# Healthcare-Robotics/mr-gan

Measured on AMD Instinct MI355X. Metric: GAN train steps/sec (labeled+unlabeled+G) at batch 4096, higher is better.
Workload: dtype bf16; 1 GPU; BASELINE configs[1]: synthetic N=65536 x D=512, K=6, batch 4096 per GPU, labeled 100/class; one step = D sub-step (3B rows) + G sub-step (2B rows) + both Adam updates; global_batch=4096, rows_per_gpu=4096, parallelism=single, batch_statistics=n/a, launch=hipGraph replay

## Files before the change

### include/mrgan_abi.h

```cpp
#ifndef MRGAN_ABI_H
#define MRGAN_ABI_H

#include <stddef.h>
#include <stdint.h>

#ifdef __cplusplus
extern "C" {
#endif

typedef struct mrgan_handle mrgan_handle;
typedef void* mrgan_stream;

enum { MRGAN_F32 = 0, MRGAN_BF16 = 1, MRGAN_FP8 = 2 };
enum { MRGAN_NET_G = 0, MRGAN_NET_D = 1 };
enum {
    MRGAN_FLAG_SYNC_STATS = 1,
    MRGAN_FLAG_FLAT_GRADS = 2,
    MRGAN_FLAG_GRAPH      = 4,
    MRGAN_FLAG_GRAD_BF16  = 8,
    MRGAN_FLAG_GAUSS_NOISE = 16
};

#define MRGAN_MAX_CLASSES 32
#define MRGAN_MAX_MODELS 16
// ... 85 lines not shown
    const float* x_unl_dev; const int32_t* idx_unl_dev;
    const float* z_dev;
    int64_t ld_x_lab, ld_x_unl;
    int64_t x_lab_model_stride, idx_lab_model_stride, labels_model_stride;
    int64_t x_unl_model_stride, idx_unl_model_stride, z_model_stride;
    int32_t stream_mode, reserved;
} mrgan_disc_group_args;
typedef struct mrgan_gen_group_args {
    const float* x_unl_dev; const int32_t* idx_unl_dev;
    const float* z_dev;
    int64_t ld_x_unl;
    int64_t x_unl_model_stride, idx_unl_model_stride, z_model_stride;
    int32_t stream_mode, reserved;
} mrgan_gen_group_args;
int mrgan_disc_step_group(mrgan_handle* h, const mrgan_disc_group_args* a, float* out3_host, mrgan_stream stream);
int mrgan_gen_step_group(mrgan_handle* h, const mrgan_gen_group_args* a, float* out1_host, mrgan_stream stream);
int mrgan_train_pair_group(mrgan_handle* h, const mrgan_disc_group_args* d, const mrgan_gen_group_args* g, mrgan_stream stream);

enum {
    MRGAN_TUNE_CHAIN = 0,
    MRGAN_TUNE_KC_CFG = 1,
    MRGAN_TUNE_KS_GROUP = 4,
    MRGAN_TUNE_PAIR_GEN = 5,
    MRGAN_TUNE_HEAD_MFMA = 6
};
int mrgan_set_tuning(mrgan_handle* h, int knob, int value);

enum {
    MRGAN_REGION_BN_STATS = 0,
    MRGAN_REGION_FM_MOMENTS = 1,
    MRGAN_REGION_BN_BWD = 2,
    MRGAN_REGION_GRAD_D = 3,
    MRGAN_REGION_GRAD_G = 4,
    MRGAN_REGION_WORKSPACE = 5,
    MRGAN_REGION_GRAD_D_BF16 = 6,
    MRGAN_REGION_GRAD_G_BF16 = 7,
    MRGAN_REGION_TAIL_D = 8,
    MRGAN_REGION_TAIL_G = 9
};
int mrgan_region(mrgan_handle* h, int region, void** ptr_dev, size_t* bytes);

int mrgan_eval_error(mrgan_handle* h, const float* x_dev, const int32_t* idx_dev, int64_t ld_x,
                     const int32_t* labels_dev, int64_t n, float* err_host, mrgan_stream stream);
int mrgan_predict_logits(mrgan_handle* h, const float* x_dev, const int32_t* idx_dev, int64_t ld_x, int64_t n,
                         float* logits_dev, mrgan_stream stream);

int mrgan_read_metrics(mrgan_handle* h, float* out8_host, int reset, mrgan_stream stream);
// ... 11 lines not shown
```

### include/mrgan_debug.h

```cpp
#ifndef MRGAN_DEBUG_H
#define MRGAN_DEBUG_H

#include "mrgan_abi.h"

#ifdef __cplusplus
extern "C" {
#endif

int mrgan_debug_noise(mrgan_handle* h, uint32_t site, uint32_t seg, uint32_t step, uint32_t row0, int rows, int cols,
                      float* out_dev, mrgan_stream stream);
int mrgan_debug_tr_probe(uint16_t* out1024_dev, mrgan_stream stream);
int mrgan_debug_ablate(mrgan_handle* h, int bits);
int mrgan_debug_buffer(mrgan_handle* h, int kind, int l, void** ptr_dev, int* rows_per_seg, int* ld, int* elem_size);
int mrgan_debug_gemm_time(int op, int m, int n, int k, int nbatch, int splits, int reps, int ablate, int kc_cfg, float* avg_us);

typedef struct mrgan_debug_gemm_desc {
    int32_t dtype, op, m, n, k, nbatch, splits;
    int32_t kchunk;
    int32_t kc_cfg;
    int32_t tune_bits;
    int32_t seg_stride, seg_rows;
    const void* a; int64_t a_bs, a_si, a_sk;
    const void* b; int64_t b_bs, b_sk, b_sj;
    int32_t act, n_valid;
    const float* bias;
    void* out; int64_t out_bs; int32_t ldo;
    float sigma; uint32_t site, seg0; int32_t seg_step; uint32_t iter_step, row0;
    uint32_t iter;
    uint64_t seed;
    uint16_t* mask; int64_t mask_bs; int32_t ldm;
    const void* h; int64_t h_bs; int32_t ldh;
    int32_t cs_mode; float* cs1; float* cs2; int32_t ldcs;
    const float* bn_mu; const float* bn_rstd;
    float* slab; int64_t slab_stride;
    void* q8; int64_t q8_bs; int32_t ldq8;
    void* q8t; int64_t q8t_bs; int32_t ldq8t;
    const void* slot_a; const void* slot_b; void* slot_o;
    int32_t gauss;
} mrgan_debug_gemm_desc;
typedef struct mrgan_debug_fold { const float* src; float* dst; int64_t stride; int32_t nsrc, n, ngroups; } mrgan_debug_fold;
int mrgan_debug_gemm_launch(const mrgan_debug_gemm_desc* d, int count, int grouped, const mrgan_debug_fold* fold,
                            char* kname, int kname_len, mrgan_stream stream);

int mrgan_debug_gemm_fp8(int m, int n, int k, const float* a_dev, const float* b_dev, const float* bias_dev, int act, float scale_a,
                         float scale_b, float* out_dev, int reps, float* avg_us, int kc_cfg, mrgan_stream stream);

int mrgan_debug_quant8(const void* src, int64_t src_bs, int ld, int rows, int cols, int nb, int prow, void* dst, int64_t dst_bs, int ldd,
                       void* dstt, int64_t dstt_bs, int lddt, void* slot_dev, int fmt, mrgan_stream stream);
int mrgan_debug_fp8_update_scales(void* slots_dev, int n, mrgan_stream stream);


typedef struct mrgan_debug_stage_seg {
    const float* src; const int32_t* idx; int64_t ld;
    int32_t rows, cols, cols_pad;
    void* out; int32_t ldo;
    float sigma; uint32_t site, seg;
    int32_t gen, stream; uint32_t iter_off;
    int32_t models; int64_t src_ms, idx_ms, out_ms;
} mrgan_debug_stage_seg;
typedef struct mrgan_debug_stage_desc {
    int32_t dtype;
    mrgan_debug_stage_seg s[5]; int32_t nseg;
    uint64_t seed; uint32_t row0;
// ... 95 lines not shown
```

### mr_gan_amd/csrc/engine_debug.hip

```cpp
#include "engine_internal.h"

namespace mrgan {
int launch_tr_probe(unsigned short* out, hipStream_t s);
}

namespace {

template <typename T>
__global__ void to_f32_kernel(const T* src, long lds, float* dst, long ldd, int rows, int cols) {
    const int c = blockIdx.x * 64 + (threadIdx.x & 63), r = blockIdx.y * 4 + (threadIdx.x >> 6);
    if (r >= rows || c >= cols) return;
    dst[(long)r * ldd + c] = Elem<T>::to_f32(src[(long)r * lds + c]);
}

}

extern "C" {

int mrgan_debug_noise(mrgan_handle* h, uint32_t site, uint32_t seg, uint32_t step, uint32_t row0, int rows, int cols, float* out,
                      mrgan_stream stream) {
    if (!h || !out) return fail(-1, "null argument");
    if (h->gauss && (row0 & 1u)) return fail(-1, "debug_noise: a true-Gaussian handle draws row pairs, row0 must be even");
    CHK(launch_noise_debug(h->gauss, h->cfg.seed, site, seg, step, row0, rows, cols, out, (hipStream_t)stream));
    return 0;
// ... 211 lines not shown
        if (d.h && (d.ldh < d.n || (bf && (d.ldh % 8)))) return fail(-1, "debug_gemm_launch: ldh");
        if (d.mask && d.ldm < d.n) return fail(-1, "debug_gemm_launch: ldm >= n");
    }
    return 0;
}

int mrgan_debug_gemm_launch(const mrgan_debug_gemm_desc* d, int count, int grouped, const mrgan_debug_fold* fold,
                            char* kname, int kname_len, mrgan_stream stream) {
    if (!d || count < 1) return fail(-1, "null argument");
    if (kname && kname_len > 0) kname[0] = 0;
    hipStream_t s = (hipStream_t)stream;
    DevState* st = nullptr;
    DevState hst[2];
    memset(hst, 0, sizeof hst);
    hst[0].iter = hst[1].iter = d[0].iter;
    HIPCHK(hipMalloc((void**)&st, sizeof hst));
    hipError_t he = hipMemcpy(st, hst, sizeof hst, hipMemcpyHostToDevice);
    const char* name = "";
    int r = he == hipSuccess ? 0 : fail(-10, "hipMemcpy failed: %s", hipGetErrorString(he));
    if (!r && !grouped) {
        GemmArgs g;
        int epi = 0;
        if (count != 1) r = fail(-1, "debug_gemm_launch: one product per plain launch");
        if (!r) r = debug_gemm_args(d[0], st, g, epi);
        if (!r) {
            r = d[0].dtype == MRGAN_FP8    ? launch_gemm_fp8(epi, g, s, &name)
                : d[0].dtype == MRGAN_BF16 ? launch_gemm_bf16(epi, g, s, &name)
                                           : launch_gemm_f32(epi, g, s, &name);
            if (r) fail(r, "debug_gemm_launch: launch refused (%d)", r);
        }
    } else if (!r) {
        GemmArgs gs[KS_GROUP_MAX];
        for (int i = 0; i < count && i < KS_GROUP_MAX && !r; ++i) {
            int epi = 0;
            r = debug_gemm_args(d[i], st, gs[i], epi);
            if (!r && (epi != EPI_SLAB || d[i].dtype != MRGAN_BF16)) r = fail(-1, "debug_gemm_launch: grouped launches are bf16 weight gradients");
        }
        FoldJob fj;
        memset(&fj, 0, sizeof fj);
        if (!r && fold) {
            if (!fold->src || !fold->dst || fold->nsrc < 1 || fold->n < 1 || fold->ngroups < 1 || fold->stride < fold->n)
                r = fail(-1, "debug_gemm_launch: fold");
            fj.src = fold->src; fj.dst = fold->dst; fj.stride = fold->stride; fj.nsrc = fold->nsrc; fj.n = fold->n; fj.ngroups = fold->ngroups;
        }
        if (!r) {
            r = launch_gemm_bf16_dw_group(gs, count, s, &name, fold ? &fj : nullptr);
            if (r < 0) fail(r, "debug_gemm_launch: grouped launch failed (%d)", r);
        }
    }
    he = hipStreamSynchronize(s);
    hipFree(st);
    if (!r && he != hipSuccess) return fail(-10, "debug_gemm_launch: %s", hipGetErrorString(he));
    if (!r && kname && kname_len > 0) snprintf(kname, (size_t)kname_len, "%s", name);
    return r;
}

int mrgan_debug_quant8(const void* src, int64_t src_bs, int ld, int rows, int cols, int nb, int prow, void* dst, int64_t dst_bs, int ldd,
                       void* dstt, int64_t dstt_bs, int lddt, void* slot, int fmt, mrgan_stream stream) {
    if (!src || rows < 0 || rows > prow || cols < 1 || cols > ld || (fmt != FP8_E4M3 && fmt != FP8_E5M2)) return fail(-1, "debug_quant8: bad argument");
    if ((dst && ldd < cols) || (dstt && (dstt_bs < 0 || lddt < (int64_t)(nb - 1) * dstt_bs + prow))) return fail(-1, "debug_quant8: ldd >= cols, lddt >= nb batches of prow bytes");
    Quant8Args a;
    memset(&a, 0, sizeof a);
    a.src = (const __bf16*)src; a.src_bs = src_bs; a.ld = ld; a.rows = rows; a.cols = cols; a.nb = nb; a.prow = prow;
    a.dst = (unsigned char*)dst; a.dst_bs = dst_bs; a.ldd = ldd;
    a.dstt = (unsigned char*)dstt; a.dstt_bs = dstt_bs; a.lddt = lddt;
    a.slot = (Fp8Slot*)slot; a.fmt = fmt;
// ... 287 lines not shown
```

### mr_gan_amd/csrc/engine_state.hip

```cpp
#include <stdarg.h>

#include "engine_internal.h"

namespace mrgan {

thread_local std::string g_err;
int fail(int code, const char* fmt, ...) {
    char buf[512];
    va_list ap;
    va_start(ap, fmt);
    vsnprintf(buf, sizeof buf, fmt, ap);
    va_end(ap);
    g_err = buf;
    return code;
}

void set_gen_view(mrgan_handle* h, int seg) {
    h->g[1].q.xseg = seg;
    const int N1p = h->g[0].Np;
    h->zbuf = rowptr(h, h->zbuf_all, (long)seg * h->S, h->nzp);
    h->h1 = rowptr(h, h->h1_all, (long)seg * h->S, N1p);
    h->hbn = rowptr(h, h->hbn_all, (long)seg * h->S, N1p);
    h->h2 = rowptr(h, h->h2_all, (long)seg * h->S, h->g[1].Np);
    h->bn_mu = h->bn_mu_all + (size_t)seg * N1p;
// ... 449 lines not shown
    HIPCHK(hipStreamSynchronize((hipStream_t)stream));
    *it = st.iter;
    return 0;
}

int mrgan_set_iterations(mrgan_handle* h, uint32_t iterations, uint32_t batch_counter, mrgan_stream stream) {
    if (!h) return fail(-1, "null handle");
    hipLaunchKernelGGL(init_state_kernel, dim3(1), dim3(1), 0, (hipStream_t)stream, h->state, iterations, batch_counter,
                       h->cfg.lr, h->cfg.beta1, h->cfg.beta2);
    return 0;
}

int mrgan_set_tuning(mrgan_handle* h, int knob, int value) {
    if (!h) return fail(-1, "null handle");
    if (h->graph_exec) { hipGraphExecDestroy(h->graph_exec); h->graph_exec = nullptr; h->graph_ready = false; }
    switch (knob) {
        case MRGAN_TUNE_CHAIN: h->use_chain = value != 0 && h->chain_ok; break;
        case MRGAN_TUNE_KC_CFG:
            if (!kc_cfg_supported(value)) return fail(-1, "unsupported forward / dX tile config %d", value);
            h->tune_kc_cfg = value; break;
        case MRGAN_TUNE_KS_GROUP: h->tune_bits = (h->tune_bits & ~TUNE_BIT_NO_KS_GROUP) | (value ? 0 : TUNE_BIT_NO_KS_GROUP); break;
        case MRGAN_TUNE_PAIR_GEN: h->tune_pair_gen = value ? 1 : 0; break;
        case MRGAN_TUNE_HEAD_MFMA: h->head_wide = value != 0 && h->head_wide_ok; break;
        default: return fail(-1, "unknown tuning knob %d", knob);
    }
    return 0;
}

int mrgan_pair_hint(mrgan_handle* h, int on) {
    if (!h) return fail(-1, "null handle");
    h->pair_gen = on ? 1 : 0;
    return 0;
}

int mrgan_region(mrgan_handle* h, int region, void** ptr, size_t* bytes) {
    if (!h || !ptr || !bytes) return fail(-1, "null argument");
    const size_t n1 = (size_t)h->g[0].Np;
    switch (region) {
        case MRGAN_REGION_BN_STATS: *ptr = h->r_bn_stats; *bytes = 4 * n1 * 4; break;
        case MRGAN_REGION_FM_MOMENTS: *ptr = h->r_fm; *bytes = 2 * (size_t)h->Fp * 4; break;
        case MRGAN_REGION_BN_BWD: *ptr = h->r_bn_bwd; *bytes = 2 * n1 * 4; break;
        case MRGAN_REGION_GRAD_D: case MRGAN_REGION_GRAD_G: {
            if (h->flat16_d) return fail(-3, "region %d: the gradients of this handle travel as bfloat16 (MRGAN_FLAG_GRAD_BF16): "
                                             "all-reduce MRGAN_REGION_GRAD_*_BF16 and MRGAN_REGION_TAIL_*", region);
            const bool d = region == MRGAN_REGION_GRAD_D;
            *ptr = d ? h->flat_d : h->flat_g; *bytes = ((d ? h->flat_d_n : h->flat_g_n) + 4) * 4;
// ... 28 lines not shown
```

### mr_gan_amd/csrc/gemm.h

```cpp
#pragma once
#include <string.h>

#include <algorithm>

#include "common.h"

namespace mrgan {

enum { EPI_FWD = 0, EPI_DX = 1, EPI_SLAB = 2 };
enum { VAR_ACT_MASK = 3, VAR_NOISE = 4, VAR_MASK = 8, VAR_GAUSS = 16, VAR_DYN = 64 };


struct Epi {
    int act;
    int n_valid;
    const float* bias;
    void* out; long out_bs; int ldo;
    float sigma; uint32_t site; uint32_t seg0;
    int seg_step; uint32_t iter_step;
    uint32_t row0;
    uint64_t seed;
    int gauss;
    uint16_t* mask; long mask_bs; int ldm;
    const void* h; long h_bs; int ldh;
    int cs_mode; float* cs1; float* cs2; int ldcs;
    const float* bn_mu; const float* bn_rstd;
    float* slab; long slab_stride;
    const DevState* st;
// ... 344 lines not shown
                        const int c = wn * wcols + ni * 32 + lc;
                        lds[(wm * 2 + 0) * bn + c] = cs1[0][ni];
                        lds[(wm * 2 + 1) * bn + c] = cs2[0][ni];
                    }
                }
                __syncthreads();
                const int t = threadIdx.x;
                if (t < bn) {
                    float s1 = 0.f, s2 = 0.f;
#pragma unroll
                    for (int w = 0; w < WM; ++w) { s1 += lds[(w * 2 + 0) * bn + t]; s2 += lds[(w * 2 + 1) * bn + t]; }
                    if (col_blk + t < g.N && col_blk + t < e.ldcs) {
                        cs1p[prow0 * e.ldcs + col_blk + t] = s1;
                        if (e.cs_mode != CS_SUM) cs2p[prow0 * e.ldcs + col_blk + t] = s2;
                    }
                }
            }
        }
        EPI_STAMP(3);
    }
#undef EPI_STAMP
}

enum { TUNE_BIT_NO_KS_GROUP = 4 };
inline bool kc_cfg_supported(int cfg) {
    return cfg == -1 || cfg == 0 || cfg == 1 || cfg == 3 || cfg == 5 || cfg == 7 || cfg == 9;
}
constexpr int KS_GROUP_MAX = 6;
struct FoldJob { const float* src; float* dst; long stride; int nsrc, n, ngroups, blocks_x; long model_stride; };
struct KsGroup {
    int n;
    int blk_end[KS_GROUP_MAX];
    FoldJob fold;
    GemmArgs g[KS_GROUP_MAX];
};

int launch_gemm_f32(int epi, const GemmArgs& g, hipStream_t s, const char** kname = nullptr);
int launch_gemm_bf16(int epi, const GemmArgs& g, hipStream_t s, const char** kname = nullptr);
int launch_gemm_fp8(int epi, const GemmArgs& g, hipStream_t s, const char** kname = nullptr);
int launch_to_fp8(const float* src, long ld_src, unsigned char* dst, long ld_dst, int rows, int cols, int prow, int pcol, float scale,
                  int transpose, hipStream_t s);
struct Quant8Args {
    const __bf16* src; long src_bs; int ld; int rows, cols, nb;
    int prow;
    unsigned char* dst; long dst_bs; int ldd;
    unsigned char* dstt; long dstt_bs; int lddt;
    Fp8Slot* slot; int fmt;
};
int launch_quant8(const Quant8Args& a, hipStream_t s);
int launch_fp8_update_scales(Fp8Slot* slots, int n, hipStream_t s);
int launch_fp8_init_slots(Fp8Slot* slots, int n, const float* targets_dev, hipStream_t s);
int launch_gemm_bf16_dw_group(const GemmArgs* gs, int n, hipStream_t s, const char** kname = nullptr,
                              const FoldJob* fold = nullptr);

constexpr int GEMM_NO_HOLES = 1 << 30;
inline GemmArgs gemm_args(int M, int N, int K, int nbatch, int tile_rows) {
    GemmArgs g;
    memset(&g, 0, sizeof g);
// ... 64 lines not shown
```

### mr_gan_amd/csrc/gemm_bf16.hip

```cpp
#include <algorithm>
#include <cstring>
#include <string>

#include "gemm.h"
#include "lds_ring.h"

namespace mrgan {

namespace {
constexpr int BN = 128, BK = RING_BK;
constexpr int KS_PITCH = 320;
constexpr int KS_TILE_BYTES = 64 * KS_PITCH;

#ifdef MRGAN_STAMPS
struct KcStamps { unsigned long long acc[6], prev, epi[5]; };
#define KC_STAMPS_PARAM , KcStamps& stamps_
#define KC_STAMPS_ARG , stamps_
#else
#define KC_STAMPS_PARAM
#define KC_STAMPS_ARG
#endif
template <int EPI, int BM, int BNT, int WM, int WN, int NS, int VAR>
__device__ __forceinline__ void kc_tile(const GemmArgs& g, const int batch , const int model, const int tile_m, const int tile_n, char* lds KC_STAMPS_PARAM) {
    constexpr int NW = WM * WN;
// ... 131 lines not shown
    static const std::string name = "gemm_bf16_kc_kernel<" + std::to_string(EPI) + ", " + std::to_string(BM) + ", " +
                                    std::to_string(BNT) + ", " + std::to_string(WM) + ", " + std::to_string(WN) + ", " +
                                    std::to_string(NS) + ", " + std::to_string(VAR) + ">";
    g_last_kernel = name.c_str();
    constexpr int STAGE = BM * 128 + BNT * 128;
    constexpr int OUT = BM * BNT * 2 + 4 * WM * BNT * 4;
    constexpr int LDS = (NS * STAGE > OUT ? NS * STAGE : OUT) + ((EPI == EPI_DX && (VAR & VAR_ACT_MASK) != ACT_RELU) ? BM * BNT * 2 : 0);
    const int tiles = ceil_div(g.M, BM) * ceil_div(g.N, BNT) * g.nbatch;
    return launch_with_dyn_lds<gemm_bf16_kc_kernel<EPI, BM, BNT, WM, WN, NS, VAR>, LDS>(dim3(persistent_grid(tiles, LDS)), dim3(64 * WM * WN), s, g);
}

__device__ __forceinline__ bf16x8 ks_frag_swz(const char* tile, int fb, int ks, int lane) {
    const int g4 = lane >> 4, i16 = lane & 15, q = i16 >> 2, p = i16 & 3;
    const int f0 = fb + (g4 & 1) * 16;
    const int m0 = ks * 16 + (g4 >> 1) * 8;
    const char* a0 = tile + (m0 + q) * 256 + ((((f0 >> 3) + (p >> 1)) ^ (q << 2)) << 4) + ((p & 1) << 3);
    const s16x4 t0 = __builtin_amdgcn_ds_read_tr16_b64_v4i16((lds_s16x4*)a0);
    const s16x4 t1 = __builtin_amdgcn_ds_read_tr16_b64_v4i16((lds_s16x4*)(a0 + 4 * 256));
    const s16x8 tt = __builtin_shufflevector(t0, t1, 0, 1, 2, 3, 4, 5, 6, 7);
    return __builtin_bit_cast(bf16x8, tt);
}

template <int NS, int WM, int WN>
__device__ __forceinline__ void ks_fast_body(const GemmArgs& g, const int bid, const int model ) {
    constexpr int NW = WM * WN;
    constexpr int MR = 128 / WM / 32, NR = 128 / WN / 32;
    constexpr int T_BYTES = 64 * 256, STAGE = 2 * T_BYTES;
    constexpr int T_INSTR = 16 / NW;
    static_assert(MR >= 1 && NR >= 1 && T_INSTR >= 1, "tile/wave layout");
    extern __shared__ __attribute__((aligned(16))) char lds[];

    const int t = threadIdx.x, lane = t & 63;
    const int wave = __builtin_amdgcn_readfirstlane(t >> 6);
    const int wm = wave / WN, wn = wave % WN;
    const int ntn = (g.N + 127) / 128, ntm = (g.M + 127) / 128;
    const int tidx = xcd_tile(bid, ntn * ntm * g.splits);
    const int split = tidx / (ntn * ntm), rem = tidx - split * (ntn * ntm);
    int tile_m, tile_n;
    if ((ntm & 7) == 0 && ntn >= 16) {
        const int grp = rem / (8 * ntn), in = rem - grp * (8 * ntn);
        tile_m = grp * 8 + (in & 7); tile_n = in >> 3;
    } else { tile_m = rem / ntn; tile_n = rem - tile_m * ntn; }
    const int row_blk = tile_m * 128, col_blk = tile_n * 128;
    const int k_begin = split * g.kchunk;
    const int k_end = (g.e.ablate & 4) ? k_begin : min(g.K, k_begin + g.kchunk);

    const __amdgpu_buffer_rsrc_t rsA = __builtin_amdgcn_make_buffer_rsrc((void*)model_ptr(g.A, g.e, model), 0, (int)((long)g.K * g.a_sk * 2), 0x00020000);
    const __amdgpu_buffer_rsrc_t rsB = __builtin_amdgcn_make_buffer_rsrc((void*)model_ptr(g.B, g.e, model), 0, (int)((long)g.K * g.b_sk * 2), 0x00020000);
    const int lrow = lane >> 4, lp = lane & 15;
    int voffA[T_INSTR], voffB[T_INSTR];
#pragma unroll
    for (int i = 0; i < T_INSTR; ++i) {
        const int kr = (wave * T_INSTR + i) * 4 + lrow;
        const int c = lp ^ ((kr & 3) << 2);
        voffA[i] = (int)(((long)kr * g.a_sk + row_blk + c * 8) * 2);
        voffB[i] = (int)(((long)kr * g.b_sk + col_blk + c * 8) * 2);
    }
    auto issue = [&](int k0, int buf) {
        char* a_dst = lds + buf * STAGE + wave * T_INSTR * 1024;
        char* b_dst = a_dst + T_BYTES;
#pragma unroll
        for (int i = 0; i < T_INSTR; ++i) glds16(rsA, a_dst + i * 1024, voffA[i], (int)((long)k0 * g.a_sk * 2));
#pragma unroll
        for (int i = 0; i < T_INSTR; ++i) glds16(rsB, b_dst + i * 1024, voffB[i], (int)((long)k0 * g.b_sk * 2));
    };
// ... 3 lines not shown
    for (int i = 0; i < MR; ++i)
#pragma unroll
        for (int j = 0; j < NR; ++j)
#pragma unroll
            for (int r = 0; r < 16; ++r) acc[i][j][r] = 0.f;

    const int nk = (k_end - k_begin + BK - 1) / BK;
#pragma unroll
    for (int p = 0; p < NS - 1; ++p)
        if (p < nk) issue(k_begin + p * BK, p);
#define KS_FRAG_A(As, mi, ks) ks_frag_swz(As, (wm * MR + mi) * 32, ks, lane)
#define KS_FRAG_B(Bs, ni, ks) ks_frag_swz(Bs, (wn * NR + ni) * 32, ks, lane)
#define KS_NO_STAMP(i)
    RING_MAINLOOP(NS, 2 * T_INSTR, MR, NR, nk, acc, issue, k_begin, KS_FRAG_A, KS_FRAG_B, lds, STAGE, T_BYTES, KS_NO_STAMP)
#undef KS_FRAG_A
#undef KS_FRAG_B
#undef KS_NO_STAMP
    __syncthreads();
    epilogue<__bf16, EPI_SLAB, MR, NR, WM>(acc, g, 0, model, split, tile_m, row_blk, col_blk, wm, wn, lane, (float*)lds, BN);
}

template <int NS, int WM, int WN>
__global__ __launch_bounds__(64 * WM * WN) void gemm_bf16_ks_fast_kernel(const GemmArgs g) {
    ks_fast_body<NS, WM, WN>(g, blockIdx.x, blockIdx.y);
}

template <int NS, int WM, int WN>
__global__ __launch_bounds__(64 * WM * WN) void gemm_bf16_ks_group_kernel(const KsGroup grp) {
    const int ngemm = grp.blk_end[grp.n - 1];
    if ((int)blockIdx.x >= ngemm) {
        const FoldJob& f = grp.fold;
        const float* fsrc = (const float*)((const char*)f.src + (long)blockIdx.y * f.model_stride);
        float* fdst = (float*)((char*)f.dst + (long)blockIdx.y * f.model_stride);
        const int fb = (int)blockIdx.x - ngemm, gidx = fb / f.blocks_x;
        const int i = (fb - gidx * f.blocks_x) * 256 + (int)threadIdx.x;
        if (threadIdx.x >= 256 || i >= f.n) return;
        float s0 = 0.f, s1 = 0.f, s2 = 0.f, s3 = 0.f;
        int p = gidx;
        for (; p + 3 * f.ngroups < f.nsrc; p += 4 * f.ngroups) {
            s0 += fsrc[(long)p * f.stride + i]; s1 += fsrc[(long)(p + f.ngroups) * f.stride + i];
            s2 += fsrc[(long)(p + 2 * f.ngroups) * f.stride + i]; s3 += fsrc[(long)(p + 3 * f.ngroups) * f.stride + i];
        }
        for (; p < f.nsrc; p += f.ngroups) s0 += fsrc[(long)p * f.stride + i];
        fdst[(long)gidx * f.stride + i] = (s0 + s1) + (s2 + s3);
        return;
    }
    int i = 0, b0 = 0;
#pragma unroll
    for (int j = 0; j < KS_GROUP_MAX - 1; ++j)
        if (j + 1 < grp.n && (int)blockIdx.x >= grp.blk_end[j]) { i = j + 1; b0 = grp.blk_end[j]; }
    ks_fast_body<NS, WM, WN>(grp.g[i], (int)blockIdx.x - b0, blockIdx.y);
}

template <int NS, int WM, int WN>
int launch_ks_fast(const GemmArgs& g, hipStream_t s) {
    static const std::string name = "gemm_bf16_ks_fast_kernel<" + std::to_string(NS) + ", " + std::to_string(WM) + ", " + std::to_string(WN) + ">";
    g_last_kernel = name.c_str();
    constexpr int STAGE = 2 * 64 * 256;
    dim3 grid(ceil_div(g.N, 128) * ceil_div(g.M, 128) * g.splits, gemm_models(g));
    return launch_with_dyn_lds<gemm_bf16_ks_fast_kernel<NS, WM, WN>, NS * STAGE>(grid, dim3(64 * WM * WN), s, g);
}

__device__ __forceinline__ bf16x8 ks_frag(const char* tile, int fb, int ks, int lane) {
    const int g4 = lane >> 4, i16 = lane & 15, q = i16 >> 2, p = i16 & 3;
    const int f0 = fb + (g4 & 1) * 16;
    const int m0 = ks * 16 + (g4 >> 1) * 8;
    const char* a0 = tile + (m0 + q) * KS_PITCH + (f0 + 4 * p) * 2;
    const s16x4 t0 = __builtin_amdgcn_ds_read_tr16_b64_v4i16((lds_s16x4*)a0);
    const s16x4 t1 = __builtin_amdgcn_ds_read_tr16_b64_v4i16((lds_s16x4*)(a0 + 4 * KS_PITCH));
    const s16x8 tt = __builtin_shufflevector(t0, t1, 0, 1, 2, 3, 4, 5, 6, 7);
    return __builtin_bit_cast(bf16x8, tt);
}

__global__ __launch_bounds__(256) void gemm_bf16_ks_kernel(const GemmArgs g) {
// ... 125 lines not shown
            case ACT_SOFTPLUS: return launch_kc_tile<EPI_FWD, ACT_SOFTPLUS>(g, s);
            default: return -3;
        }
    }
    switch (var) {
        case ACT_RELU: return launch_kc_tile<EPI_DX, ACT_RELU>(g, s);
        case ACT_SOFTPLUS: return launch_kc_tile<EPI_DX, ACT_SOFTPLUS>(g, s);
        default: return launch_kc_tile<EPI_DX, ACT_LINEAR>(g, s);
    }
}

static bool ks_dense_k(const GemmArgs& g) {
    return g.a_si == 1 && g.b_sj == 1 && gemm_model_batches(g) == 1 && (g.K % BK) == 0 && (g.kchunk % BK) == 0 &&
           (g.seg_rows >= g.seg_stride || g.K <= g.seg_rows) &&
           (long)g.K * g.a_sk * 2 < (1L << 31) && (long)g.K * g.b_sk * 2 < (1L << 31);
}

int launch_gemm_bf16_dw_group(const GemmArgs* gs, int n, hipStream_t s, const char** kname, const FoldJob* fold) {
    if (n < 1 || n > KS_GROUP_MAX) return 1;
    if (gs[0].e.tune_bits & TUNE_BIT_NO_KS_GROUP) return 1;
    KsGroup grp;
    memset(&grp, 0, sizeof grp);
    grp.n = n;
    int total = 0;
    const int models = gemm_models(gs[0]);
    for (int i = 0; i < n; ++i) {
        if (!ks_dense_k(gs[i]) || gemm_models(gs[i]) != models) return 1;
        const int blocks = ceil_div(gs[i].N, 128) * ceil_div(gs[i].M, 128) * gs[i].splits;
        total += blocks;
        grp.blk_end[i] = total;
        grp.g[i] = gs[i];
    }
    if (fold && fold->n > 0) {
        grp.fold = *fold;
        grp.fold.blocks_x = ceil_div(fold->n, 256);
        total += grp.fold.blocks_x * fold->ngroups;
    }
    constexpr int STAGE = 2 * 64 * 256, LDS = 2 * STAGE;
    if (const int r = launch_with_dyn_lds<gemm_bf16_ks_group_kernel<2, 2, 4>, LDS>(dim3(total, models), dim3(512), s, grp)) return r;
    if (kname) *kname = "gemm_bf16_ks_group_kernel<2, 2, 4>";
    return hipGetLastError() == hipSuccess ? 0 : -2;
}

int launch_gemm_bf16(int epi, const GemmArgs& g, hipStream_t s, const char** kname) {
    int r = 0;
    if (epi == EPI_SLAB) {
        if (g.a_si != 1 || g.b_sj != 1) return -3;
        if (ks_dense_k(g)) {
            r = launch_ks_fast<3, 2, 4>(g, s);
        } else {
            dim3 grid(ceil_div(g.N, BN), ceil_div(g.M, 128), g.nbatch * g.splits);
            MRGAN_LAUNCH(gemm_bf16_ks_kernel, grid, dim3(256), 0, s, g);
            g_last_kernel = "gemm_bf16_ks_kernel";
        }
    } else {
        if (g.a_sk != 1 || g.b_sk != 1 || g.splits != 1 || (g.K % BK) != 0) return -3;
        if ((long)g.M * g.a_si * 2 >= (1L << 31) || (long)g.N * g.b_sj * 2 >= (1L << 31)) return -3;
        r = launch_kc_any(epi, g, s);
    }
    if (r) return r;
// ... 11 lines not shown
```

### mr_gan_amd/engine.py

```python
import ctypes as C
import os

import numpy as np
import torch

_HERE = os.path.dirname(os.path.abspath(__file__))
LIB_PATH = os.path.join(_HERE, "lib", "libmrgan_hip.so")

F32, BF16, FP8 = 0, 1, 2
NET_G, NET_D = 0, 1
FLAG_SYNC_STATS, FLAG_FLAT_GRADS, FLAG_GRAPH, FLAG_GRAD_BF16, FLAG_GAUSS_NOISE = 1, 2, 4, 8, 16
NOISE_MODES = ('irwin-hall', 'gaussian')
D_GEN, D_MAIN, D_ADAM = 0, 1, 2
G_GEN, G_FEAT, G_BWD, G_TAIL, G_ADAM = 0, 1, 2, 3, 4
TUNE_CHAIN, TUNE_KC_CFG, TUNE_KS_GROUP, TUNE_PAIR_GEN, TUNE_HEAD_MFMA = 0, 1, 4, 5, 6
REGION_BN_STATS, REGION_FM_MOMENTS, REGION_BN_BWD, REGION_GRAD_D, REGION_GRAD_G, REGION_WORKSPACE = range(6)
REGION_GRAD_D_BF16, REGION_GRAD_G_BF16, REGION_TAIL_D, REGION_TAIL_G = 6, 7, 8, 9

EXPORTS = [
    "mrgan_default_config", "mrgan_workspace_bytes", "mrgan_create", "mrgan_destroy", "mrgan_last_error",
    "mrgan_num_tensors", "mrgan_tensor_shape", "mrgan_set_weights", "mrgan_get_weights", "mrgan_get_slot",
    "mrgan_set_slot", "mrgan_get_iterations", "mrgan_set_iterations", "mrgan_disc_step", "mrgan_gen_step",
    "mrgan_train_pair", "mrgan_sup_step", "mrgan_fp8_calibration", "mrgan_logmel", "mrgan_logmel_frames", "mrgan_region", "mrgan_eval_error", "mrgan_predict_logits", "mrgan_read_metrics",
    "mrgan_pair_hint", "mrgan_set_tuning", "mrgan_debug_noise", "mrgan_debug_tr_probe", "mrgan_debug_gemm_launch", "mrgan_profile_begin", "mrgan_profile_end", "mrgan_debug_ablate", "mrgan_debug_gemm_time", "mrgan_debug_buffer", "mrgan_debug_gemm_fp8",
    "mrgan_debug_quant8", "mrgan_debug_fp8_update_scales",
    "mrgan_debug_stage", "mrgan_debug_reduce_partials","mrgan_debug_colsum_finalize", "mrgan_debug_bn_apply", "mrgan_debug_bn_bwd", "mrgan_debug_head", "mrgan_debug_head_wide",
    "mrgan_debug_fm", "mrgan_debug_adam",
    "mrgan_select_model", "mrgan_sup_step_group",
    "mrgan_disc_step_group", "mrgan_gen_step_group", "mrgan_train_pair_group",
]
MAX_MODELS = 16
PROF_NAME_LEN = 96


class Config(C.Structure):
    _fields_ = [
        ("d_in", C.c_int32), ("batch", C.c_int32), ("noise_size", C.c_int32),
        ("g_hidden", C.c_int32 * 2), ("d_hidden", C.c_int32 * 5),
# ... 404 lines not shown
        _check(self.lib.mrgan_debug_noise(self.handle, site, seg, step, row0, rows, cols, _ptr(out), _stream()))
        return out


class DebugGemmDesc(C.Structure):
    _fields_ = [
        ("dtype", C.c_int32), ("op", C.c_int32), ("m", C.c_int32), ("n", C.c_int32), ("k", C.c_int32),
        ("nbatch", C.c_int32), ("splits", C.c_int32), ("kchunk", C.c_int32), ("kc_cfg", C.c_int32), ("tune_bits", C.c_int32),
        ("seg_stride", C.c_int32), ("seg_rows", C.c_int32),
        ("a", C.c_void_p), ("a_bs", C.c_int64), ("a_si", C.c_int64), ("a_sk", C.c_int64),
        ("b", C.c_void_p), ("b_bs", C.c_int64), ("b_sk", C.c_int64), ("b_sj", C.c_int64),
        ("act", C.c_int32), ("n_valid", C.c_int32), ("bias", C.c_void_p),
        ("out", C.c_void_p), ("out_bs", C.c_int64), ("ldo", C.c_int32),
        ("sigma", C.c_float), ("site", C.c_uint32), ("seg0", C.c_uint32), ("seg_step", C.c_int32),
        ("iter_step", C.c_uint32), ("row0", C.c_uint32), ("iter", C.c_uint32), ("seed", C.c_uint64),
        ("mask", C.c_void_p), ("mask_bs", C.c_int64), ("ldm", C.c_int32),
        ("h", C.c_void_p), ("h_bs", C.c_int64), ("ldh", C.c_int32),
        ("cs_mode", C.c_int32), ("cs1", C.c_void_p), ("cs2", C.c_void_p), ("ldcs", C.c_int32),
        ("bn_mu", C.c_void_p), ("bn_rstd", C.c_void_p),
        ("slab", C.c_void_p), ("slab_stride", C.c_int64),
        ("q8", C.c_void_p), ("q8_bs", C.c_int64), ("ldq8", C.c_int32),
        ("q8t", C.c_void_p), ("q8t_bs", C.c_int64), ("ldq8t", C.c_int32),
        ("slot_a", C.c_void_p), ("slot_b", C.c_void_p), ("slot_o", C.c_void_p),
        ("gauss", C.c_int32),
    ]


class DebugFold(C.Structure):
    _fields_ = [("src", C.c_void_p), ("dst", C.c_void_p), ("stride", C.c_int64), ("nsrc", C.c_int32), ("n", C.c_int32),
                ("ngroups", C.c_int32)]


def debug_gemm_desc(**kw):
    d = DebugGemmDesc()
    d.kc_cfg, d.nbatch, d.splits = -1, 1, 1
    d._refs = []
    for name, v in kw.items():
        if isinstance(v, torch.Tensor):
            d._refs.append(v)
            v = v.data_ptr()
        setattr(d, name, v)
    return d


def debug_gemm_launch(descs, grouped=False, fold=None):
    if isinstance(descs, DebugGemmDesc):
        descs = [descs]
    arr = (DebugGemmDesc * len(descs))(*descs)
    name = C.create_string_buffer(PROF_NAME_LEN)
    f = None
    if fold is not None:
        src, dst, stride, nsrc, n, ngroups = fold
        f = DebugFold(src.data_ptr(), dst.data_ptr(), stride, nsrc, n, ngroups)
    rc = load_library().mrgan_debug_gemm_launch(arr, len(descs), 1 if grouped else 0, C.byref(f) if f is not None else None,
                                                name, PROF_NAME_LEN, _stream())
    if rc not in (0, 1, -1, -3):
        _check(rc)
    return rc, name.value.decode()


HEAD_LAB, HEAD_UNL, HEAD_FAKE, HEAD_EVAL, HEAD_LOGITS, HEAD_MSE = range(6)
ADAM_FUSED, ADAM_REDUCE_ONLY, ADAM_FROM_FLAT = range(3)


class DebugStageSeg(C.Structure):
    _fields_ = [
        ("src", C.c_void_p), ("idx", C.c_void_p), ("ld", C.c_int64),
        ("rows", C.c_int32), ("cols", C.c_int32), ("cols_pad", C.c_int32),
        ("out", C.c_void_p), ("ldo", C.c_int32),
        ("sigma", C.c_float), ("site", C.c_uint32), ("seg", C.c_uint32),
        ("gen", C.c_int32), ("stream", C.c_int32), ("iter_off", C.c_uint32),
        ("models", C.c_int32), ("src_ms", C.c_int64), ("idx_ms", C.c_int64), ("out_ms", C.c_int64),
    ]


class DebugStageDesc(C.Structure):
# ... 219 lines not shown
```

Baseline: 2645 steps/s.

## Plan grouped split-K weight-gradient blocks per XCD to balance load and L2 reuse

Adds a host-built schedule (KsPlan) for the grouped bf16 weight-gradient kernel that assigns GEMM tile pieces and fold-reduction blocks to each of the 8 XCDs. It uses a longest-first greedy balance and fills idle slots with fold blocks. The kernel decodes each block's problem, split and tile from a per-XCD segment table held in scalar registers. The aim is to cut XCD load imbalance and repeated fetching of A/B strips across XCD L2 caches. In exchange it adds decode overhead, padding with idle blocks, and a threshold heuristic that falls back to the old order.

```diff
diff --git a/include/mrgan_abi.h b/include/mrgan_abi.h
--- a/include/mrgan_abi.h
+++ b/include/mrgan_abi.h
@@ -131,7 +131,8 @@
     MRGAN_TUNE_KC_CFG = 1,
     MRGAN_TUNE_KS_GROUP = 4,
     MRGAN_TUNE_PAIR_GEN = 5,
-    MRGAN_TUNE_HEAD_MFMA = 6
+    MRGAN_TUNE_HEAD_MFMA = 6,
+    MRGAN_TUNE_KS_PLAN = 7
 };
 int mrgan_set_tuning(mrgan_handle* h, int knob, int value);
 
diff --git a/include/mrgan_debug.h b/include/mrgan_debug.h
--- a/include/mrgan_debug.h
+++ b/include/mrgan_debug.h
@@ -36,9 +36,10 @@
     void* q8; int64_t q8_bs; int32_t ldq8;
     void* q8t; int64_t q8t_bs; int32_t ldq8t;
     const void* slot_a; const void* slot_b; void* slot_o;
+    int64_t model_stride; int32_t models;
     int32_t gauss;
 } mrgan_debug_gemm_desc;
-typedef struct mrgan_debug_fold { const float* src; float* dst; int64_t stride; int32_t nsrc, n, ngroups; } mrgan_debug_fold;
+typedef struct mrgan_debug_fold { const float* src; float* dst; int64_t stride; int32_t nsrc, n, ngroups; int64_t model_stride; } mrgan_debug_fold;
 int mrgan_debug_gemm_launch(const mrgan_debug_gemm_desc* d, int count, int grouped, const mrgan_debug_fold* fold,
                             char* kname, int kname_len, mrgan_stream stream);
 
diff --git a/mr_gan_amd/csrc/engine_debug.hip b/mr_gan_amd/csrc/engine_debug.hip
--- a/mr_gan_amd/csrc/engine_debug.hip
+++ b/mr_gan_amd/csrc/engine_debug.hip
@@ -257,6 +257,7 @@
         GemmArgs g;
         int epi = 0;
         if (count != 1) r = fail(-1, "debug_gemm_launch: one product per plain launch");
+        if (!r && d[0].models > 1) r = fail(-1, "debug_gemm_launch: model groups are for grouped weight gradients");
         if (!r) r = debug_gemm_args(d[0], st, g, epi);
         if (!r) {
             r = d[0].dtype == MRGAN_FP8    ? launch_gemm_fp8(epi, g, s, &name)
@@ -270,6 +271,10 @@
             int epi = 0;
             r = debug_gemm_args(d[i], st, gs[i], epi);
             if (!r && (epi != EPI_SLAB || d[i].dtype != MRGAN_BF16)) r = fail(-1, "debug_gemm_launch: grouped launches are bf16 weight gradients");
+            if (!r && d[i].models > 1) {
+                if (d[i].nbatch != 1 || (d[i].model_stride % 16)) r = fail(-1, "debug_gemm_launch: a model group needs nbatch 1 and a model_stride of whole 16 bytes");
+                else gs[i] = gemm_group(gs[i], d[i].models, (long)d[i].model_stride);
+            }
         }
         FoldJob fj;
         memset(&fj, 0, sizeof fj);
@@ -277,6 +282,7 @@
             if (!fold->src || !fold->dst || fold->nsrc < 1 || fold->n < 1 || fold->ngroups < 1 || fold->stride < fold->n)
                 r = fail(-1, "debug_gemm_launch: fold");
             fj.src = fold->src; fj.dst = fold->dst; fj.stride = fold->stride; fj.nsrc = fold->nsrc; fj.n = fold->n; fj.ngroups = fold->ngroups;
+            fj.model_stride = (long)fold->model_stride;
         }
         if (!r) {
             r = launch_gemm_bf16_dw_group(gs, count, s, &name, fold ? &fj : nullptr);
diff --git a/mr_gan_amd/csrc/engine_state.hip b/mr_gan_amd/csrc/engine_state.hip
--- a/mr_gan_amd/csrc/engine_state.hip
+++ b/mr_gan_amd/csrc/engine_state.hip
@@ -495,6 +495,11 @@
         case MRGAN_TUNE_KS_GROUP: h->tune_bits = (h->tune_bits & ~TUNE_BIT_NO_KS_GROUP) | (value ? 0 : TUNE_BIT_NO_KS_GROUP); break;
         case MRGAN_TUNE_PAIR_GEN: h->tune_pair_gen = value ? 1 : 0; break;
         case MRGAN_TUNE_HEAD_MFMA: h->head_wide = value != 0 && h->head_wide_ok; break;
+        case MRGAN_TUNE_KS_PLAN:
+            if (value < 0 || value > 2) return fail(-1, "MRGAN_TUNE_KS_PLAN takes 0, 1 or 2, not %d", value);
+            h->tune_bits = (h->tune_bits & ~(TUNE_BIT_KS_PARENT_ORDER | TUNE_BIT_KS_PLAN_ALWAYS)) |
+                           (value == 0 ? TUNE_BIT_KS_PARENT_ORDER : value == 2 ? TUNE_BIT_KS_PLAN_ALWAYS : 0);
+            break;
         default: return fail(-1, "unknown tuning knob %d", knob);
     }
     return 0;
diff --git a/mr_gan_amd/csrc/gemm.h b/mr_gan_amd/csrc/gemm.h
--- a/mr_gan_amd/csrc/gemm.h
+++ b/mr_gan_amd/csrc/gemm.h
@@ -4,6 +4,7 @@
 #include <algorithm>
 
 #include "common.h"
+#include "ks_plan.h"
 
 namespace mrgan {
 
@@ -394,18 +395,21 @@
 #undef EPI_STAMP
 }
 
-enum { TUNE_BIT_NO_KS_GROUP = 4 };
+enum { TUNE_BIT_NO_KS_GROUP = 4, TUNE_BIT_KS_PARENT_ORDER = 8, TUNE_BIT_KS_PLAN_ALWAYS = 16 };
 inline bool kc_cfg_supported(int cfg) {
     return cfg == -1 || cfg == 0 || cfg == 1 || cfg == 3 || cfg == 5 || cfg == 7 || cfg == 9;
 }
 constexpr int KS_GROUP_MAX = 6;
 struct FoldJob { const float* src; float* dst; long stride; int nsrc, n, ngroups, blocks_x; long model_stride; };
+static_assert(KS_GROUP_MAX == KS_PLAN_PROBLEMS, "the plan's problem codes");
 struct KsGroup {
-    int n;
+    int n, ngemm;
     int blk_end[KS_GROUP_MAX];
     FoldJob fold;
+    KsPlan plan;
     GemmArgs g[KS_GROUP_MAX];
 };
+static_assert(sizeof(KsGroup) <= 4096, "KsGroup travels as the kernel's argument");
 
 int launch_gemm_f32(int epi, const GemmArgs& g, hipStream_t s, const char** kname = nullptr);
 int launch_gemm_bf16(int epi, const GemmArgs& g, hipStream_t s, const char** kname = nullptr);
diff --git a/mr_gan_amd/csrc/gemm_bf16.hip b/mr_gan_amd/csrc/gemm_bf16.hip
--- a/mr_gan_amd/csrc/gemm_bf16.hip
+++ b/mr_gan_amd/csrc/gemm_bf16.hip
@@ -177,7 +177,8 @@
 }
 
 template <int NS, int WM, int WN>
-__device__ __forceinline__ void ks_fast_body(const GemmArgs& g, const int bid, const int model ) {
+__device__ __forceinline__ void ks_fast_body(const GemmArgs& g, const int split, const int tile_m, const int tile_n,
+                                             const int model ) {
     constexpr int NW = WM * WN;
     constexpr int MR = 128 / WM / 32, NR = 128 / WN / 32;
     constexpr int T_BYTES = 64 * 256, STAGE = 2 * T_BYTES;
@@ -188,14 +189,6 @@
     const int t = threadIdx.x, lane = t & 63;
     const int wave = __builtin_amdgcn_readfirstlane(t >> 6);
     const int wm = wave / WN, wn = wave % WN;
-    const int ntn = (g.N + 127) / 128, ntm = (g.M + 127) / 128;
-    const int tidx = xcd_tile(bid, ntn * ntm * g.splits);
-    const int split = tidx / (ntn * ntm), rem = tidx - split * (ntn * ntm);
-    int tile_m, tile_n;
-    if ((ntm & 7) == 0 && ntn >= 16) {
-        const int grp = rem / (8 * ntn), in = rem - grp * (8 * ntn);
-        tile_m = grp * 8 + (in & 7); tile_n = in >> 3;
-    } else { tile_m = rem / ntn; tile_n = rem - tile_m * ntn; }
     const int row_blk = tile_m * 128, col_blk = tile_n * 128;
     const int k_begin = split * g.kchunk;
     const int k_end = (g.e.ablate & 4) ? k_begin : min(g.K, k_begin + g.kchunk);
@@ -245,34 +238,58 @@
 
 template <int NS, int WM, int WN>
 __global__ __launch_bounds__(64 * WM * WN) void gemm_bf16_ks_fast_kernel(const GemmArgs g) {
-    ks_fast_body<NS, WM, WN>(g, blockIdx.x, blockIdx.y);
+    int split, tile_m, tile_n;
+    ks_parent_tile((int)blockIdx.x, (g.M + 127) / 128, (g.N + 127) / 128, g.splits, split, tile_m, tile_n);
+    ks_fast_body<NS, WM, WN>(g, split, tile_m, tile_n, blockIdx.y);
+}
+
+__device__ __forceinline__ void ks_fold_block(const FoldJob& f, const int fb, const int model) {
+    const float* fsrc = (const float*)((const char*)f.src + (long)model * f.model_stride);
+    float* fdst = (float*)((char*)f.dst + (long)model * f.model_stride);
+    const int gidx = fb / f.blocks_x;
+    const int i = (fb - gidx * f.blocks_x) * 256 + (int)threadIdx.x;
+    if (threadIdx.x >= 256 || i >= f.n) return;
+    float s0 = 0.f, s1 = 0.f, s2 = 0.f, s3 = 0.f;
+    int p = gidx;
+    for (; p + 3 * f.ngroups < f.nsrc; p += 4 * f.ngroups) {
+        s0 += fsrc[(long)p * f.stride + i]; s1 += fsrc[(long)(p + f.ngroups) * f.stride + i];
+        s2 += fsrc[(long)(p + 2 * f.ngroups) * f.stride + i]; s3 += fsrc[(long)(p + 3 * f.ngroups) * f.stride + i];
+    }
+    for (; p < f.nsrc; p += f.ngroups) s0 += fsrc[(long)p * f.stride + i];
+    fdst[(long)gidx * f.stride + i] = (s0 + s1) + (s2 + s3);
 }
 
 template <int NS, int WM, int WN>
 __global__ __launch_bounds__(64 * WM * WN) void gemm_bf16_ks_group_kernel(const KsGroup grp) {
-    const int ngemm = grp.blk_end[grp.n - 1];
-    if ((int)blockIdx.x >= ngemm) {
-        const FoldJob& f = grp.fold;
-        const float* fsrc = (const float*)((const char*)f.src + (long)blockIdx.y * f.model_stride);
-        float* fdst = (float*)((char*)f.dst + (long)blockIdx.y * f.model_stride);
-        const int fb = (int)blockIdx.x - ngemm, gidx = fb / f.blocks_x;
-        const int i = (fb - gidx * f.blocks_x) * 256 + (int)threadIdx.x;
-        if (threadIdx.x >= 256 || i >= f.n) return;
-        float s0 = 0.f, s1 = 0.f, s2 = 0.f, s3 = 0.f;
-        int p = gidx;
-        for (; p + 3 * f.ngroups < f.nsrc; p += 4 * f.ngroups) {
-            s0 += fsrc[(long)p * f.stride + i]; s1 += fsrc[(long)(p + f.ngroups) * f.stride + i];
-            s2 += fsrc[(long)(p + 2 * f.ngroups) * f.stride + i]; s3 += fsrc[(long)(p + 3 * f.ngroups) * f.stride + i];
-        }
-        for (; p < f.nsrc; p += f.ngroups) s0 += fsrc[(long)p * f.stride + i];
-        fdst[(long)gidx * f.stride + i] = (s0 + s1) + (s2 + s3);
-        return;
-    }
-    int i = 0, b0 = 0;
-#pragma unroll
-    for (int j = 0; j < KS_GROUP_MAX - 1; ++j)
-        if (j + 1 < grp.n && (int)blockIdx.x >= grp.blk_end[j]) { i = j + 1; b0 = grp.blk_end[j]; }
-    ks_fast_body<NS, WM, WN>(grp.g[i], (int)blockIdx.x - b0, blockIdx.y);
+    static_assert(KS_GROUP_MAX == 6 && KS_PLAN_SEGS == 16, "operands of the pin");
+    uint32_t row[KS_PLAN_SEGS];
+#pragma unroll
+    for (int j = 0; j < KS_PLAN_SEGS; ++j) row[j] = grp.plan.seg[blockIdx.x & (KS_PLAN_XCDS - 1)][j];
+    int on = grp.plan.on, n = grp.n, ngemm = grp.ngemm;
+    int be[KS_GROUP_MAX - 1];
+#pragma unroll
+    for (int j = 0; j < KS_GROUP_MAX - 1; ++j) be[j] = grp.blk_end[j];
+    asm volatile("" : "+s"(row[0]), "+s"(row[1]), "+s"(row[2]), "+s"(row[3]), "+s"(row[4]), "+s"(row[5]), "+s"(row[6]), "+s"(row[7]),
+                      "+s"(row[8]), "+s"(row[9]), "+s"(row[10]), "+s"(row[11]), "+s"(row[12]), "+s"(row[13]), "+s"(row[14]), "+s"(row[15]),
+                      "+s"(on), "+s"(n), "+s"(ngemm), "+s"(be[0]), "+s"(be[1]), "+s"(be[2]), "+s"(be[3]), "+s"(be[4]));
+    int i = 0, split, tile_m, tile_n, tile;
+    ks_plan_decode_row(row, (int)blockIdx.x >> 3, i, split, tile);
+    if (on) {
+        if (i == KS_PLAN_IDLE) return;
+        if (i == KS_PLAN_FOLD) { ks_fold_block(grp.fold, tile, blockIdx.y); return; }
+        const int ntn = (grp.g[i].N + 127) / 128;
+        tile_m = tile / ntn; tile_n = tile - tile_m * ntn;
+    } else {
+        if ((int)blockIdx.x >= ngemm) { ks_fold_block(grp.fold, (int)blockIdx.x - ngemm, blockIdx.y); return; }
+        int b0 = 0;
+        i = 0;
+#pragma unroll
+        for (int j = 0; j < KS_GROUP_MAX - 1; ++j)
+            if (j + 1 < n && (int)blockIdx.x >= be[j]) { i = j + 1; b0 = be[j]; }
+        const GemmArgs& g = grp.g[i];
+        ks_parent_tile((int)blockIdx.x - b0, (g.M + 127) / 128, (g.N + 127) / 128, g.splits, split, tile_m, tile_n);
+    }
+    ks_fast_body<NS, WM, WN>(grp.g[i], split, tile_m, tile_n, blockIdx.y);
 }
 
 template <int NS, int WM, int WN>
@@ -444,20 +461,29 @@
     KsGroup grp;
     memset(&grp, 0, sizeof grp);
     grp.n = n;
-    int total = 0;
+    int total = 0, fold_blocks = 0;
     const int models = gemm_models(gs[0]);
+    KsPlanProblem pp[KS_GROUP_MAX];
     for (int i = 0; i < n; ++i) {
         if (!ks_dense_k(gs[i]) || gemm_models(gs[i]) != models) return 1;
-        const int blocks = ceil_div(gs[i].N, 128) * ceil_div(gs[i].M, 128) * gs[i].splits;
-        total += blocks;
+        pp[i] = KsPlanProblem{ceil_div(gs[i].M, 128), ceil_div(gs[i].N, 128), gs[i].splits};
+        total += pp[i].ntm * pp[i].ntn * pp[i].splits;
         grp.blk_end[i] = total;
         grp.g[i] = gs[i];
     }
+    grp.ngemm = total;
     if (fold && fold->n > 0) {
         grp.fold = *fold;
         grp.fold.blocks_x = ceil_div(fold->n, 256);
-        total += grp.fold.blocks_x * fold->ngroups;
-    }
+        fold_blocks = grp.fold.blocks_x * fold->ngroups;
+        total += fold_blocks;
+    }
+    const int tb = gs[0].e.tune_bits;
+    if (!(tb & TUNE_BIT_KS_PARENT_ORDER) && ks_plan_build(pp, n, fold_blocks, models, grp.plan) &&
+        ((tb & TUNE_BIT_KS_PLAN_ALWAYS) || 2 * KS_PLAN_XCDS * grp.plan.slots <= 3 * total))
+        total = KS_PLAN_XCDS * grp.plan.slots;
+    else
+        grp.plan.on = 0;
     constexpr int STAGE = 2 * 64 * 256, LDS = 2 * STAGE;
     if (const int r = launch_with_dyn_lds<gemm_bf16_ks_group_kernel<2, 2, 4>, LDS>(dim3(total, models), dim3(512), s, grp)) return r;
     if (kname) *kname = "gemm_bf16_ks_group_kernel<2, 2, 4>";
diff --git a/mr_gan_amd/csrc/ks_plan.h b/mr_gan_amd/csrc/ks_plan.h
--- /dev/null
+++ b/mr_gan_amd/csrc/ks_plan.h
@@ -0,0 +1,188 @@
+#pragma once
+#include <stddef.h>
+#include <stdint.h>
+
+#include <vector>
+
+#if defined(__HIPCC__)
+#define KS_PLAN_HD __host__ __device__ __forceinline__
+#else
+#define KS_PLAN_HD inline
+#endif
+
+namespace mrgan {
+
+constexpr int KS_PLAN_XCDS = 8;
+constexpr int KS_PLAN_SLOTS = 64;
+constexpr int KS_PLAN_SEGS = 16;
+constexpr int KS_PLAN_PROBLEMS = 6;
+enum { KS_PLAN_FOLD = 6, KS_PLAN_IDLE = 7 };
+
+struct KsPlanProblem { int ntm, ntn, splits; };
+struct KsPlanBlock { int problem, split, tile_m, tile_n, tile; };
+
+struct KsPlan {
+    int on;
+    int slots;
+    uint32_t seg[KS_PLAN_XCDS][KS_PLAN_SEGS];
+};
+
+KS_PLAN_HD uint32_t ks_plan_run(int slot, int problem, int split, int tile) {
+    return (uint32_t)slot | ((uint32_t)problem << 7) | ((uint32_t)split << 10) | ((uint32_t)tile << 16);
+}
+
+KS_PLAN_HD void ks_plan_decode_row(const uint32_t* row, int j, int& problem, int& split, int& tile) {
+    uint32_t e = row[0];
+#if defined(__HIPCC__)
+#pragma unroll
+#endif
+    for (int i = 1; i < KS_PLAN_SEGS; ++i) {
+        const uint32_t c = row[i];
+        if ((int)(c & 127u) <= j) e = c;
+    }
+    problem = (int)((e >> 7) & 7u); split = (int)((e >> 10) & 63u);
+    tile = (int)(e >> 16) + j - (int)(e & 127u);
+}
+KS_PLAN_HD void ks_plan_decode(const KsPlan& plan, int b, int& problem, int& split, int& tile) {
+    ks_plan_decode_row(plan.seg[b & (KS_PLAN_XCDS - 1)], b >> 3, problem, split, tile);
+}
+
+KS_PLAN_HD void ks_parent_tile(int bid, int ntm, int ntn, int splits, int& split, int& tile_m, int& tile_n) {
+    const int nt = ntn * ntm * splits;
+    const int tidx = (nt & 7) == 0 ? (bid & 7) * (nt >> 3) + (bid >> 3) : bid;
+    split = tidx / (ntn * ntm);
+    const int rem = tidx - split * (ntn * ntm);
+    if ((ntm & 7) == 0 && ntn >= 16) {
+        const int grp = rem / (8 * ntn), in = rem - grp * (8 * ntn);
+        tile_m = grp * 8 + (in & 7); tile_n = in >> 3;
+    } else { tile_m = rem / ntn; tile_n = rem - tile_m * ntn; }
+}
+
+inline bool ks_plan_build(const KsPlanProblem* p, int n, int fold_blocks, int models, KsPlan& plan) {
+    plan.on = 0; plan.slots = 0;
+    for (int x = 0; x < KS_PLAN_XCDS; ++x)
+        for (int i = 0; i < KS_PLAN_SEGS; ++i) plan.seg[x][i] = ks_plan_run(0, KS_PLAN_IDLE, 0, 0);
+    if (n < 1 || n > KS_PLAN_PROBLEMS || models < 1 || fold_blocks < 0) return false;
+    const int cap = KS_PLAN_SLOTS / models;
+    if (cap < 1) return false;
+    struct Piece { int problem, split, first, count; };
+    constexpr int MAXP = KS_PLAN_XCDS * KS_PLAN_SEGS;
+    Piece pc[MAXP];
+    int np = 0;
+    for (int i = 0; i < n; ++i) {
+        const int tiles = p[i].ntm * p[i].ntn;
+        if (p[i].ntm < 1 || p[i].ntn < 1 || p[i].splits < 1 || p[i].splits > 64 || tiles >= 65536) return false;
+        int rows = p[i].ntm;
+        if (tiles > cap) {
+            const int fit = cap / p[i].ntn;
+            if (fit < 1) return false;
+            const int pieces = (p[i].ntm + fit - 1) / fit;
+            rows = (p[i].ntm + pieces - 1) / pieces;
+        }
+        for (int s = 0; s < p[i].splits; ++s)
+            for (int r = 0; r < p[i].ntm; r += rows) {
+                if (np == MAXP) return false;
+                const int nr = p[i].ntm - r < rows ? p[i].ntm - r : rows;
+                pc[np++] = Piece{i, s, r * p[i].ntn, nr * p[i].ntn};
+            }
+    }
+    for (int a = 1; a < np; ++a) {
+        const Piece v = pc[a];
+        int b = a;
+        for (; b > 0 && pc[b - 1].count < v.count; --b) pc[b] = pc[b - 1];
+        pc[b] = v;
+    }
+    int load[KS_PLAN_XCDS] = {0}, nseg[KS_PLAN_XCDS] = {0};
+    auto add = [&](int x, int problem, int split, int first, int count) {
+        if (nseg[x] == KS_PLAN_SEGS) return false;
+        plan.seg[x][nseg[x]++] = ks_plan_run(load[x], problem, split, first);
+        load[x] += count;
+        return true;
+    };
+    for (int a = 0; a < np; ++a) {
+        int x = 0;
+        for (int y = 1; y < KS_PLAN_XCDS; ++y) if (load[y] < load[x]) x = y;
+        if (load[x] + pc[a].count > cap) return false;
+        if (!add(x, pc[a].problem, pc[a].split, pc[a].first, pc[a].count)) return false;
+    }
+    int slots = 0;
+    for (int x = 0; x < KS_PLAN_XCDS; ++x) slots = load[x] > slots ? load[x] : slots;
+    int fb = 0;
+    for (int x = 0; x < KS_PLAN_XCDS && fb < fold_blocks; ++x) {
+        const int idle = slots - load[x], take = idle < fold_blocks - fb ? idle : fold_blocks - fb;
+        if (take > 0) { if (!add(x, KS_PLAN_FOLD, 0, fb, take)) return false; fb += take; }
+    }
+    if (fb < fold_blocks) {
+        const int rest = fold_blocks - fb, q = rest / KS_PLAN_XCDS, r = rest % KS_PLAN_XCDS;
+        for (int x = 0; x < KS_PLAN_XCDS; ++x) {
+            const int take = q + (x < r ? 1 : 0);
+            if (take > 0) { if (!add(x, KS_PLAN_FOLD, 0, fb, take)) return false; fb += take; }
+        }
+        slots += q + (r ? 1 : 0);
+    }
+    if (slots < 1 || slots > cap) return false;
+    for (int x = 0; x < KS_PLAN_XCDS; ++x) {
+        if (load[x] == slots) continue;
+        if (nseg[x] == KS_PLAN_SEGS) return false;
+        for (int i = nseg[x]; i < KS_PLAN_SEGS; ++i) plan.seg[x][i] = ks_plan_run(load[x], KS_PLAN_IDLE, 0, 0);
+    }
+    for (int x = 0; x < KS_PLAN_XCDS; ++x)
+        if (load[x] == slots)
+            for (int i = nseg[x]; i < KS_PLAN_SEGS; ++i) plan.seg[x][i] = ks_plan_run(127, KS_PLAN_IDLE, 0, 0);
+    plan.slots = slots; plan.on = 1;
+    return true;
+}
+
+inline int ks_parent_blocks(const KsPlanProblem* p, int n, int fold_blocks) {
+    int total = fold_blocks;
+    for (int i = 0; i < n; ++i) total += p[i].ntm * p[i].ntn * p[i].splits;
+    return total;
+}
+
+inline KsPlanBlock ks_block_of(const KsPlan* plan, const KsPlanProblem* p, int n, int fold_blocks, int b) {
+    KsPlanBlock k = {KS_PLAN_IDLE, 0, 0, 0, 0};
+    if (plan && plan->on) {
+        ks_plan_decode(*plan, b, k.problem, k.split, k.tile);
+        if (k.problem < KS_PLAN_PROBLEMS) { k.tile_m = k.tile / p[k.problem].ntn; k.tile_n = k.tile - k.tile_m * p[k.problem].ntn; }
+        return k;
+    }
+    int b0 = 0;
+    for (int i = 0; i < n; ++i) {
+        const int blocks = p[i].ntm * p[i].ntn * p[i].splits;
+        if (b < b0 + blocks) {
+            k.problem = i;
+            ks_parent_tile(b - b0, p[i].ntm, p[i].ntn, p[i].splits, k.split, k.tile_m, k.tile_n);
+            k.tile = k.tile_m * p[i].ntn + k.tile_n;
+            return k;
+        }
+        b0 += blocks;
+    }
+    if (b < b0 + fold_blocks) { k.problem = KS_PLAN_FOLD; k.tile = b - b0; }
+    return k;
+}
+
+inline double ks_fetch_bytes(const KsPlan* plan, const KsPlanProblem* p, const double* strip_bytes, int n, int fold_blocks, int models) {
+    const int gx = plan && plan->on ? KS_PLAN_XCDS * plan->slots : ks_parent_blocks(p, n, fold_blocks);
+    double bytes = 0.0;
+    for (int x = 0; x < KS_PLAN_XCDS; ++x)
+        for (int y = 0; y < models; ++y) {
+            std::vector<std::vector<char> > seen(n);
+            for (int i = 0; i < n; ++i) seen[i].assign((size_t)p[i].splits * (p[i].ntm + p[i].ntn), 0);
+            for (int b = 0; b < gx; ++b) {
+                if (((b + y * gx) & (KS_PLAN_XCDS - 1)) != x) continue;
+                const KsPlanBlock k = ks_block_of(plan, p, n, fold_blocks, b);
+                if (k.problem >= KS_PLAN_PROBLEMS) continue;
+                char* s = &seen[k.problem][(size_t)k.split * (p[k.problem].ntm + p[k.problem].ntn)];
+                if (!s[k.tile_m]) { s[k.tile_m] = 1; bytes += strip_bytes[k.problem]; }
+                if (!s[p[k.problem].ntm + k.tile_n]) { s[p[k.problem].ntm + k.tile_n] = 1; bytes += strip_bytes[k.problem]; }
+            }
+        }
+    return bytes;
+}
+inline double ks_ideal_bytes(const KsPlanProblem* p, const double* strip_bytes, int n, int models) {
+    double bytes = 0.0;
+    for (int i = 0; i < n; ++i) bytes += (double)models * p[i].splits * (p[i].ntm + p[i].ntn) * strip_bytes[i];
+    return bytes;
+}
+
+}
diff --git a/mr_gan_amd/engine.py b/mr_gan_amd/engine.py
--- a/mr_gan_amd/engine.py
+++ b/mr_gan_amd/engine.py
@@ -13,7 +13,7 @@
 NOISE_MODES = ('irwin-hall', 'gaussian')
 D_GEN, D_MAIN, D_ADAM = 0, 1, 2
 G_GEN, G_FEAT, G_BWD, G_TAIL, G_ADAM = 0, 1, 2, 3, 4
-TUNE_CHAIN, TUNE_KC_CFG, TUNE_KS_GROUP, TUNE_PAIR_GEN, TUNE_HEAD_MFMA = 0, 1, 4, 5, 6
+TUNE_CHAIN, TUNE_KC_CFG, TUNE_KS_GROUP, TUNE_PAIR_GEN, TUNE_HEAD_MFMA, TUNE_KS_PLAN = 0, 1, 4, 5, 6, 7
 REGION_BN_STATS, REGION_FM_MOMENTS, REGION_BN_BWD, REGION_GRAD_D, REGION_GRAD_G, REGION_WORKSPACE = range(6)
 REGION_GRAD_D_BF16, REGION_GRAD_G_BF16, REGION_TAIL_D, REGION_TAIL_G = 6, 7, 8, 9
 
@@ -464,13 +464,14 @@
         ("q8", C.c_void_p), ("q8_bs", C.c_int64), ("ldq8", C.c_int32),
         ("q8t", C.c_void_p), ("q8t_bs", C.c_int64), ("ldq8t", C.c_int32),
         ("slot_a", C.c_void_p), ("slot_b", C.c_void_p), ("slot_o", C.c_void_p),
+        ("model_stride", C.c_int64), ("models", C.c_int32),
         ("gauss", C.c_int32),
     ]
 
 
 class DebugFold(C.Structure):
     _fields_ = [("src", C.c_void_p), ("dst", C.c_void_p), ("stride", C.c_int64), ("nsrc", C.c_int32), ("n", C.c_int32),
-                ("ngroups", C.c_int32)]
+                ("ngroups", C.c_int32), ("model_stride", C.c_int64)]
 
 
 def debug_gemm_desc(**kw):
@@ -492,8 +493,8 @@
     name = C.create_string_buffer(PROF_NAME_LEN)
     f = None
     if fold is not None:
-        src, dst, stride, nsrc, n, ngroups = fold
-        f = DebugFold(src.data_ptr(), dst.data_ptr(), stride, nsrc, n, ngroups)
+        src, dst, stride, nsrc, n, ngroups = fold[:6]
+        f = DebugFold(src.data_ptr(), dst.data_ptr(), stride, nsrc, n, ngroups, fold[6] if len(fold) > 6 else 0)
     rc = load_library().mrgan_debug_gemm_launch(arr, len(descs), 1 if grouped else 0, C.byref(f) if f is not None else None,
                                                 name, PROF_NAME_LEN, _stream())
     if rc not in (0, 1, -1, -3):
```

After: 2646 steps/s, median of 2. About the same (+0.0%).
